# nlesc-smcm/hymls

Measured on AMD Instinct MI355X. Metric: Preconditioner ApplyInverse DoF/s + achieved HBM GB/s, Stokes3D, higher is better.
Workload: dtype f64

## Files before the change

hymls_amd/csrc/device.hpp:

```cpp
#pragma once
#include <cstdio>
#include "common.hpp"
#include "symbolic.hpp"

namespace hymls {
namespace dev {

struct Context;
Context* create_context(int device);
void bind(Context* c);
Context* current();
void destroy_context(Context* c);
void* stream();
const double* zeros16();
void* alloc(size_t bytes);
void free(void* p);
void h2d(void* dst, const void* src, size_t bytes);
void d2h(void* dst, const void* src, size_t bytes);
void d2d(void* dst, const void* src, size_t bytes);
void zero(void* dst, size_t bytes);
void sync();
size_t mem_free();
void* shared_scratch(size_t bytes);
constexpr int NSIDE = 8;
inline int side_streams() {
  static const int n = std::getenv("HYMLS_MI_SIDE_STREAMS") ? std::max(1, std::min(NSIDE, std::atoi(std::getenv("HYMLS_MI_SIDE_STREAMS")))) : 4;
  return n;
}
void fork_streams();
void use_stream(int k);
void join_streams();
void range_push(const char* label);
void range_pop();
struct Range {
  Range(const char* cls, int level, const char* fn) {
    char buf[96];
    std::snprintf(buf, sizeof buf, "%s_L%d: %s", cls, level, fn);
    range_push(buf);
  }
  ~Range() { range_pop(); }
  Range(const Range&) = delete;
  Range& operator=(const Range&) = delete;
};
void timer_start(int id);
double timer_stop(int id);
void mark(int phase, bool begin);
void profile_collect(double* sum, int* cnt);

template <class T, class A>
T* upload(const std::vector<T, A>& v) {
  T* p = (T*)alloc(std::max<size_t>(v.size(), 1) * sizeof(T));
  if (!v.empty()) h2d(p, v.data(), v.size() * sizeof(T));
  return p;
}

struct FrontD {
  int32_t c0, w, ri, rs;
  int32_t parent, idx_off, rel_off, c_off, a_off, lf_off;
  int32_t ent_begin, ent_end, child_begin, child_end;
  int64_t f_off, lp_off, q_off;
  int32_t pair = 0;
};

struct alignas(16) FwRec { int32_t item; uint16_t n; uint16_t s[5]; };

struct PlanD {
  int32_t nI, nS, nfronts, nent;
  const FrontD* fronts;
  const int32_t* fidx;
  const int32_t* rel;
  const int32_t* children;
  const int32_t* ent_id;
  const int32_t* ent_pos;
  const double* ent_w;
  const int32_t* asm_ptr;
  const int32_t* asm_src;
  int32_t asm_rows;
  const int32_t* fw_ptr;
  const int32_t* fw_items;
  const struct FwRec* fw_rec;
  const int32_t* bw_ptr;
  const int32_t* bw_items;
  int32_t nlev, max_level_rows;
  int32_t s_ent_begin, s_ent_end;
  int64_t scratch_size, factor_size;
  int32_t contrib_size;
  int32_t max_solve_rows;
  int32_t packed;
};

struct BatchD {
  int32_t nb;
  const int32_t* src;
  const int32_t* xoff;
  double* factor;
  double* scratch;
  double* sblock;
  double* contrib;
  int32_t* flag;
  double* tmp;
  int64_t tmp_stride;
  double* swork;
  int64_t swork_stride;
};

void gather(int64_t n, const int32_t* idx, const double* src, double* dst);
void scatter(int64_t n, const int32_t* idx, const double* src, double* dst);
void scatter_add(int64_t n, const int32_t* idx, const double* src, double* dst);
void axpby(int64_t n, double a, const double* x, double b, double* y);
void scale_copy(int64_t n, double a, const double* x, double* y);
inline int spmv_lanes(int32_t nrows, int64_t nnz_hint) {
  const double avg = nnz_hint >= 0 ? (double)nnz_hint / nrows : 8.0;
  return avg < 2.5 ? 1 : (avg < 5.0 ? 2 : (avg < 20.0 ? 4 : 8));
}
void spmv(int32_t nrows, const int32_t* rowptr, const int32_t* col, const double* val,
          const double* x, double* y, double alpha, double beta, int64_t nnz_hint = -1);
void spmv_mv(int32_t nrows, const int32_t* rowptr, const int32_t* col, const double* val, const double* x, int64_t ldx,
             double* y, int64_t ldy, int nv, double alpha, double beta, int64_t nnz_hint = -1);
void pull_sum(int64_t n, const int64_t* ptr, const int64_t* idx, const double* in, double* out);
void offdiag_count(int64_t nrows, const int32_t* rows, const int32_t* krow, const int32_t* kcol, const int32_t* ta, const int32_t* tb,
                   const int32_t* excl, int32_t* count);
void offdiag_fill(int64_t nrows, const int32_t* rows, const int32_t* krow, const int32_t* kcol, const int32_t* ta, const int32_t* tb,
                  const int32_t* excl, const int32_t* rowptr, int32_t* col, int32_t* src);
void member_sources(int32_t nb, int32_t next, int32_t nent, const int32_t* ext, const int32_t* ent_row, const int32_t* ent_col,
                    const int32_t* krow, const int32_t* kcol, int32_t* src, int32_t* flag);
void build_pull_tables(int64_t nrows, const int64_t* rcount, const int32_t* rowptr, const uint64_t* keys, int64_t* ptr, int64_t* idx);
void pull_sum_blocks(int64_t blen, int32_t nblk, const int64_t* ptr, const int64_t* base,
                     const double* in, double* out);

void factor_level(const PlanD& P, const BatchD& B, const int32_t* list, int32_t count,
                  int32_t b0, int32_t nbc, const double* kval, int32_t max_w);
void sblock_init(const PlanD& P, const BatchD& B, int32_t b0, int32_t nbc, const double* kval);

constexpr int PIECE = 128;
void factor_big_front(const PlanD& P, const BatchD& B, const FrontD& F, const FrontD* kids, int32_t nkids,
                      int32_t b0, int32_t nbc, const double* kval);
void root_update(const PlanD& P, const BatchD& B, const FrontD& F, int32_t nbc);
inline int solve_kt() {
  static const int kt = (std::getenv("HYMLS_MI_SOLVE_KT") && std::atoi(std::getenv("HYMLS_MI_SOLVE_KT")) == 1024) ? 1024 : 256;
  return kt;
}
void solve_fwd_big(const PlanD& P, const BatchD& B, const int32_t* list, const FrontD* hfronts, const int64_t* poff,
                   int32_t count, double* x);
void solve_bwd_big(const PlanD& P, const BatchD& B, const int32_t* list, const FrontD* hfronts, const int64_t* poff,
                   int32_t count, double* x);

void solve_fwd_level(const PlanD& P, const BatchD& B, const int32_t* list, int32_t count, double* x);
void solve_bwd_level(const PlanD& P, const BatchD& B, const int32_t* list, int32_t count, double* x);

#if defined(__HIPCC__)
#define HYMLS_HD __host__ __device__
#else
#define HYMLS_HD
#endif
HYMLS_HD inline int64_t packed_lower(int64_t w, int64_t i, int64_t k) { return k * (2 * w - k - 1) / 2 + (i - k - 1); }
HYMLS_HD inline int64_t packed_l21(int64_t w, int64_t ri, int64_t i, int64_t k) { return w * (w - 1) / 2 + i + ri * k; }
HYMLS_HD inline int64_t packed_upper(int64_t w, int64_t ri, int64_t i, int64_t k) { return w * (w - 1) / 2 + ri * w + k * (k + 1) / 2 + i; }
constexpr int32_t PAIR_L = 1, PAIR_Q = 2;
HYMLS_HD inline int64_t paired_cols(int64_t ld, int64_t ncol, int64_t i, int64_t k) {
  return k < (ncol & ~(int64_t)1) ? 2 * (ld * (k >> 1) + i) + (k & 1) : ld * k + i;
}
HYMLS_HD inline int64_t paired_lower(int64_t w, int64_t i, int64_t k) {
  const int64_t j = k >> 1;
  return i >= 2 * j + 2 ? 2 * j * (w - 1 - j) + 2 * (i - 2 * j - 2) + (k & 1) : w * (w - 1) / 2 - w / 2 + j;
}
HYMLS_HD inline int64_t paired_l21(int64_t w, int64_t ri, int64_t i, int64_t k) { return w * (w - 1) / 2 + paired_cols(ri, w, i, k); }
HYMLS_HD inline int64_t paired_q(int64_t w, int64_t ri, int64_t i, int64_t k) { return paired_cols(w, ri, i, k); }
void repack_fronts(const PlanD& P, const BatchD& B, int32_t b0, int32_t nbc);

struct FusedSub {
  union {
    const double* fac;
    const float* fac32;
  };
  int32_t xoff;
  int32_t cls;
};
constexpr int FUSED_MAX_ITEMS = 2048;
struct FusedIO {
  int32_t in = 0, out = 0, a_lanes = 1;
  const double* b = nullptr; const int32_t* perm = nullptr;
  const int32_t* a_row = nullptr; const int32_t* a_col = nullptr; const double* a_val = nullptr; const double* x2 = nullptr;
  const double* z = nullptr; double* user = nullptr;
};
void interior_solve_fused(int32_t nsub, const FusedSub* subs, const PlanD* plans, int32_t lds_doubles, double* x,
                          const FusedIO* io = nullptr);

constexpr int32_t FLAG_F32_RANGE = 4;
void demote_panels(int64_t n, const double* src, float* dst, int32_t* flag);
void round_panels(int64_t n, double* slab, int32_t* flag);
void interior_solve_fused_f32(int32_t nsub, const FusedSub* subs, const PlanD* plans, int32_t lds_doubles, double* x,
                              const FusedIO* io = nullptr);

struct LvlSub {
  union {
    const double* fac;
    const float* fac32;
  };
  double* contrib; int32_t xoff, cls;
  int64_t cstride;
};
struct LvlTask { int32_t sub, front, r0, pad; };
constexpr int LVL_MAX_ROWS = 6144;
constexpr int LVL_SMALL_ROWS = 256;
void solve_fwd_tasks(const LvlTask* tasks, int32_t ntasks, const LvlSub* subs, const PlanD* plans, int32_t lds_doubles,
                     const double* x, double* y);
void solve_bwd_tasks(const LvlTask* tasks, int32_t ntasks, const LvlSub* subs, const PlanD* plans, int32_t lds_doubles,
                     const double* y, double* x);

constexpr int NV_MAX = 4;
void interior_solve_fused_mv(int32_t nsub, const FusedSub* subs, const PlanD* plans, int32_t lds_doubles, int32_t front_doubles,
                             double* x, int64_t ldx, int nv);
void interior_solve_fused_mv_f32(int32_t nsub, const FusedSub* subs, const PlanD* plans, int32_t lds_doubles, int32_t front_doubles,
                                 double* x, int64_t ldx, int nv);
void solve_fwd_tasks_mv(const LvlTask* tasks, int32_t ntasks, const LvlSub* subs, const PlanD* plans, int32_t lds_doubles,
                        const double* x, double* y, int64_t ld, int nv);
void solve_bwd_tasks_mv(const LvlTask* tasks, int32_t ntasks, const LvlSub* subs, const PlanD* plans, int32_t lds_doubles,
                        const double* y, double* x, int64_t ld, int nv);
void solve_fwd_tasks_mv_f32(const LvlTask* tasks, int32_t ntasks, const LvlSub* subs, const PlanD* plans, int32_t lds_doubles,
                            const double* x, double* y, int64_t ld, int nv);
void solve_bwd_tasks_mv_f32(const LvlTask* tasks, int32_t ntasks, const LvlSub* subs, const PlanD* plans, int32_t lds_doubles,
                            const double* y, double* x, int64_t ld, int nv);

void ot_apply(int32_t ng, const int32_t* gptr, const double* w, double* x);
void sblock_transform(int32_t nS, int32_t ng, const int32_t* gptr, const double* tv,
                      double* sblock, int32_t nbc);
void sblock_extract(int32_t nS, int64_t npick, const int32_t* pick, const double* sblock,
                    double* out, int64_t out_stride, int32_t nbc);
struct KeptD {
  int32_t nS, ngl;
  const int32_t* gptr; const int32_t* glink; const int32_t* goff; const int64_t* lboff; const int32_t* lblen;
};
void sblock_kept(const KeptD& K, const double* tv, const double* sblock, double* out, int64_t out_stride, int32_t nbc);
bool sblock_kept_fits(int32_t nS, int32_t ngl);
void dense_invert(int32_t nb, int32_t nblk, double* blocks, int32_t* flag);
bool dense_invert_blocked_order(int32_t nb);
void blocks_apply(int32_t nb, int32_t nblk, const double* binv, const int32_t* ids,
                  const double* x, double* y);

double dot(int64_t n, const double* x, const double* y);
void solve_transposed(const PlanD& P, const BatchD& B, const int32_t* order, int32_t nfronts, int32_t max_rows, double* x);
// ... 9 lines not shown
```

hymls_amd/csrc/device_hip.hip:

```cpp
#include <hip/hip_runtime.h>
#include <type_traits>
#include <dlfcn.h>
#include <chrono>
#include <cstring>
#include <cfloat>
#include <array>
#include <map>
#include <string>
#include <cstdio>
#include "device.hpp"

namespace hymls {
namespace dev {

#define HIP_CHECK(call)                                                                    \
  do {                                                                                     \
    hipError_t e_ = (call);                                                                \
    if (e_ != hipSuccess)                                                                  \
      throw ::hymls::Error(-3, std::string("HIP error: ") + hipGetErrorString(e_) + " at " + \
                                   __FILE__ + ":" + std::to_string(__LINE__));             \
  } while (0)

struct MarkRec { int phase; bool begin; hipEvent_t ev; };
struct Context {
// ... 2179 lines not shown
  const bool pl = (F.pair & PAIR_L) != 0, pq = (F.pair & PAIR_Q) != 0;
  double* Q = B.factor + (int64_t)b * P.factor_size + F.q_off;
  for (int64_t t = threadIdx.x; t < n; t += 256) tmp[t] = Lp[t];
  if (pq) for (int64_t t = threadIdx.x; t < w * ri; t += 256) tmp[n + t] = Q[t];
  __syncthreads();
  for (int64_t t = threadIdx.x; t < n; t += 256) {
    const int64_t i = t % ld, k = t / ld;
    const int64_t dst = i >= w ? (pl ? paired_l21(w, ri, i - w, k) : packed_l21(w, ri, i - w, k))
                               : (i > k ? (pl ? paired_lower(w, i, k) : packed_lower(w, i, k)) : packed_upper(w, ri, i, k));
    Lp[dst] = tmp[t];
  }
  if (pq) for (int64_t t = threadIdx.x; t < w * ri; t += 256) Q[paired_q(w, ri, t % w, t / w)] = tmp[n + t];
}
void repack_fronts(const PlanD& P, const BatchD& B, int32_t b0, int32_t nbc) {
  if (P.nfronts <= 0 || nbc <= 0) return;
  hipLaunchKernelGGL(k_repack, dim3(P.nfronts, nbc), dim3(256), 0, g_stream, P, B, b0);
  launch_check();
}

__global__ void __launch_bounds__(256) k_demote_panels(const double* __restrict__ src, float* __restrict__ dst, int64_t n, int64_t head,
                                                        int32_t* __restrict__ flag) {
  const int64_t tid = (int64_t)blockIdx.x * 256 + threadIdx.x, nthr = (int64_t)gridDim.x * 256;
  bool bad = false;
  auto cv = [&](double v) { bad |= !(fabs(v) <= (double)FLT_MAX); return (float)v; };
  const int64_t nq = (n - head) / 4;
  const double2* s2 = (const double2*)(src + head);
  float4* d4 = (float4*)(dst + head);
  for (int64_t q = tid; q < nq; q += nthr) {
    const double2 a = s2[2 * q], b = s2[2 * q + 1];
    d4[q] = make_float4(cv(a.x), cv(a.y), cv(b.x), cv(b.y));
  }
  for (int64_t t = tid; t < head; t += nthr) dst[t] = cv(src[t]);
  for (int64_t t = head + 4 * nq + tid; t < n; t += nthr) dst[t] = cv(src[t]);
  if (bad) atomicOr(flag, FLAG_F32_RANGE);
}
void demote_panels(int64_t n, const double* src, float* dst, int32_t* flag) {
  if (n <= 0) return;
  int64_t head = std::min<int64_t>(n, (int64_t)(((16 - (uintptr_t)dst % 16) % 16) / sizeof(float)));
  if ((uintptr_t)(src + head) % 16 != 0) head = n;
  hipLaunchKernelGGL(k_demote_panels, dim3(nblocks(std::max<int64_t>(n / 4, 1), 256, 8192)), dim3(256), 0, g_stream, src, dst, n, head, flag);
  launch_check();
}
__global__ void __launch_bounds__(256) k_round_panels(double* __restrict__ slab, int64_t n, int32_t* __restrict__ flag) {
  bool bad = false;
  for (int64_t t = (int64_t)blockIdx.x * 256 + threadIdx.x; t < n; t += (int64_t)gridDim.x * 256) {
    const double v = slab[t];
    bad |= !(fabs(v) <= (double)FLT_MAX);
    slab[t] = (double)(float)v;
  }
  if (bad) atomicOr(flag, FLAG_F32_RANGE);
}
void round_panels(int64_t n, double* slab, int32_t* flag) {
  if (n <= 0) return;
  hipLaunchKernelGGL(k_round_panels, dim3(nblocks(n, 256, 8192)), dim3(256), 0, g_stream, slab, n, flag);
  launch_check();
}

struct FusedFront { int32_t c0, w, ri, c_off, a_off, lf_off, idx_off, pad; int64_t lp_off, q_off; };
template <class PTR>
__device__ inline PTR lside_pair(PTR base, int r, int w, int ri, int& c1, int& tri, PTR& ps) {
  const int low = (w * (w - 1)) >> 1;
  if (r < w) { c1 = 2 * (w - 3); tri = 1; ps = base + (low - (w >> 1) + ((r - 1) >> 1)); return base + (2 * r - 4); }
  c1 = 2 * ri; tri = 0; ps = base + (low + ri * (w - 1) + (r - w));
  return base + (low + 2 * (r - w));
}
template <class PTR>
__device__ inline PTR lside(PTR base, int packed, int r, int w, int ri, int& c1, int& tri) {
  if (!packed) { c1 = w + ri; tri = 0; return base + r; }
  if (r < w) { c1 = w; tri = 1; return base + (r - 1); }
  c1 = ri; tri = 0;
  return base + ((w * (w - 1)) >> 1) + (r - w);
}
template <class PTR>
__device__ inline PTR uside(PTR base, int packed, int i, int w, int ri, int& c1, int& tri) {
  if (!packed) { c1 = w + ri; tri = 0; return base + i; }
  c1 = 0; tri = 1;
  return base + ((w * (w - 1)) >> 1) + ri * w + i;
}
template <int L>
__device__ __forceinline__ void fused_spmv_rows(int n, int tid, gptr<int32_t> rp, gptr<int32_t> col, gptr<double> val, gptr<double> x, double* y) {
  const int lane = tid % L, rpb = 256 / L;
  for (int base = 0; base < n; base += 4 * rpb) {
    int k[4], e[4], c[4];
    double a[4], xv[4];
#pragma unroll
    for (int j = 0; j < 4; j++) {
      const int row = base + j * rpb + tid / L;
      k[j] = 0; e[j] = 0;
      if (row < n) { k[j] = rp[row] + lane; e[j] = rp[row + 1]; }
    }
#pragma unroll
    for (int j = 0; j < 4; j++) { a[j] = 0.0; c[j] = 0; if (k[j] < e[j]) { a[j] = val[k[j]]; c[j] = col[k[j]]; } }
#pragma unroll
    for (int j = 0; j < 4; j++) { xv[j] = 0.0; if (k[j] < e[j]) xv[j] = x[c[j]]; }
#pragma unroll
    for (int j = 0; j < 4; j++) {
      if (base + j * rpb >= n) break;
      const int row = base + j * rpb + tid / L;
      double s = 0.0;
      if (k[j] < e[j]) {
        s += a[j] * xv[j];
        for (int kk = k[j] + L; kk < e[j]; kk += L) s += val[kk] * x[col[kk]];
      }
#pragma unroll
      for (int off = L / 2; off > 0; off >>= 1) s += __shfl_down(s, off, L);
      if (row < n && lane == 0) y[row] = s + 0.0;
    }
  }
}
template <bool PROF, class PT, int IN, int OUT>
__device__ __forceinline__ void interior_fused_body(const FusedSub* __restrict__ subs, const PlanD* __restrict__ plans,
                                                    double* __restrict__ x, long long* __restrict__ prof, const FusedIO io) {
  extern __shared__ double lds[];
  auto ldp = [](gptr<PT> q) { return (double)*q; };
  long long tp[6] = {0, 0, 0, 0, 0, 0}, t0 = 0, tstart = 0;
  auto tick = [&](int bucket) { if (PROF) { const long long t = wall_clock64(); tp[bucket] += t - t0; t0 = t; } };
  if (PROF) { t0 = wall_clock64(); tstart = t0; }
  const FusedSub S = subs[blockIdx.x];
  const PlanD P = plans[S.cls];
  double* X = lds;
  double* C = lds + P.nI;
  double* Fv = C + P.contrib_size;
  double* R = Fv + 128;
  FusedFront* LF = (FusedFront*)(Fv + (P.max_level_rows > 384 ? P.max_level_rows : 384));
  const int tid = threadIdx.x;
  for (int i = tid; i < P.nfronts; i += 256) {
    const FrontD G = P.fronts[i];
    FusedFront f;
    f.c0 = G.c0; f.w = G.w; f.ri = G.ri; f.c_off = G.c_off; f.a_off = G.a_off; f.lf_off = G.lf_off; f.idx_off = G.idx_off;
    f.pad = P.packed ? G.pair : 0;
    f.lp_off = G.lp_off; f.q_off = G.q_off;
    LF[i] = f;
  }
  double* xg = x + S.xoff;
  if (IN == 0) {
    for (int i = tid; i < P.nI; i += 256) X[i] = xg[i];
  } else if (IN == 1) {
    const gptr<int32_t> perm = as_global(io.perm) + S.xoff;
    const gptr<double> b = as_global(io.b);
    for (int i = tid; i < P.nI; i += 256) X[i] = b[perm[i]];
  } else {
    const gptr<int32_t> a_row = as_global(io.a_row) + S.xoff, a_col = as_global(io.a_col);
    const gptr<double> a_val = as_global(io.a_val), x2 = as_global(io.x2);
    switch (io.a_lanes) {
      case 1: fused_spmv_rows<1>(P.nI, tid, a_row, a_col, a_val, x2, X); break;
      case 2: fused_spmv_rows<2>(P.nI, tid, a_row, a_col, a_val, x2, X); break;
      case 4: fused_spmv_rows<4>(P.nI, tid, a_row, a_col, a_val, x2, X); break;
      default: fused_spmv_rows<8>(P.nI, tid, a_row, a_col, a_val, x2, X); break;
    }
  }
  __syncthreads();
  tick(0);
  const gptr<PT> fac = as_global((const PT*)(const void*)S.fac);
  const gptr<int32_t> fw_items = as_global(P.fw_items), bw_items = as_global(P.bw_items), fidx = as_global(P.fidx),
                      asm_ptr = as_global(P.asm_ptr), asm_src = as_global(P.asm_src), fw_ptr = as_global(P.fw_ptr), bw_ptr = as_global(P.bw_ptr);
  typedef int v4i __attribute__((ext_vector_type(4)));
  const gptr<v4i> fw_rec = (gptr<v4i>)P.fw_rec;
  for (int lev = 0; lev < P.nlev; lev++) {
    const int ib = fw_ptr[lev], ni = fw_ptr[lev + 1] - ib;
    for (int it = tid; it < ni; it += 256) {
      FwRec rc;
      { const v4i q = fw_rec[ib + it]; static_assert(sizeof(FwRec) == 16, "FwRec is one dwordx4"); __builtin_memcpy(&rc, &q, 16); }
      const int item = rc.item;
      const FusedFront& F = LF[item >> 16];
      const int r = item & 0xffff;
      double v = r < F.w ? X[F.c0 + r] : 0.0;
      if (rc.n != 0xffff) {
#pragma unroll
        for (int q = 0; q < 5; q++) if (q < rc.n) v += C[rc.s[q]];
      } else {
        for (int t = asm_ptr[F.a_off + r]; t < asm_ptr[F.a_off + r + 1]; t++) v += C[asm_src[t]];
      }
      if (r < F.w) Fv[F.lf_off + r] = v; else C[F.c_off + r - F.w] = v;
    }
    __syncthreads();
    tick(1);
    if (ni > 128) {
      for (int it = tid; it < ni; it += 256) {
        const int item = fw_items[ib + it];
        const FusedFront& F = LF[item >> 16];
        const int r = item & 0xffff, w = F.w;
        int c1, tri;
        const double* f = Fv + F.lf_off;
        const int kmax = r < w ? r : w;
        double a[4];
#pragma unroll
        for (int u = 0; u < 4; u++) a[u] = 0.0;
        int k = 0;
        if (F.pad & PAIR_L) {
          gptr<PT> ps;
          const gptr<PT> pp = lside_pair(fac + F.lp_off, r, w, F.ri, c1, tri, ps);
          auto pair_at = [&](int j) { return load_pair<PT>(pp + (c1 * j - tri * 2 * j * j)); };
          for (; k + 3 < kmax; k += 4) {
            const PanelPair<PT> l0 = pair_at(k >> 1), l1 = pair_at((k >> 1) + 1);
            a[0] += (double)l0.a * f[k]; a[1] += (double)l0.b * f[k + 1]; a[2] += (double)l1.a * f[k + 2]; a[3] += (double)l1.b * f[k + 3];
          }
          const bool hp = k + 1 < kmax, hs = (kmax & 1) != 0;
          PanelPair<PT> tl = {}; PT ts = 0;
          if (hp) tl = pair_at(k >> 1);
          if (hs) ts = *ps;
          if (hp) { a[0] += (double)tl.a * f[k]; a[0] += (double)tl.b * f[k + 1]; }
          if (hs) a[0] += (double)ts * f[kmax - 1];
        } else {
          const gptr<PT> p = lside(fac + F.lp_off, P.packed, r, w, F.ri, c1, tri);
          for (; k + 3 < kmax; k += 4) {
            double l[4];
#pragma unroll
            for (int u = 0; u < 4; u++) l[u] = ldp(p + (c1 * (k + u) - tri * (((k + u) * (k + u + 3)) >> 1)));
#pragma unroll
            for (int u = 0; u < 4; u++) a[u] += l[u] * f[k + u];
          }
          tail_batch<3>([&](int u) { return k + u < kmax; },
                        [&](int u) { return ldp(p + (c1 * (k + u) - tri * (((k + u) * (k + u + 3)) >> 1))); },
                        [&](int u, double l) { a[0] += l * f[k + u]; });
        }
        const double sum = (a[0] + a[1]) + (a[2] + a[3]);
        if (r < w) X[F.c0 + r] = f[r] + sum; else C[F.c_off + r - w] -= sum;
      }
    } else {
      const int RT = ni > 64 ? 128 : 64, KG = 256 / RT;
      const int it = tid % RT, kg = tid / RT;
      double a0 = 0.0, a1 = 0.0, a2 = 0.0, a3 = 0.0;
      if (it < ni) {
        const int item = fw_items[ib + it];
        const FusedFront& F = LF[item >> 16];
        const int r = item & 0xffff, w = F.w;
        int c1, tri;
        const gptr<PT> p = lside(fac + F.lp_off, P.packed, r, w, F.ri, c1, tri);
        const double* f = Fv + F.lf_off;
        const int kmax = r < w ? r : w;
        auto at = [&](int kk) { return ldp(p + (c1 * kk - tri * ((kk * (kk + 3)) >> 1))); };
        int k = kg;
        for (; k + 3 * KG < kmax; k += 4 * KG) {
          const double l0 = at(k), l1 = at(k + KG), l2 = at(k + 2 * KG), l3 = at(k + 3 * KG);
          a0 += l0 * f[k]; a1 += l1 * f[k + KG]; a2 += l2 * f[k + 2 * KG]; a3 += l3 * f[k + 3 * KG];
        }
        tail_batch<3>([&](int u) { return k + u * KG < kmax; }, [&](int u) { return at(k + u * KG); },
                      [&](int u, double l) { a0 += l * f[k + u * KG]; });
      }
      R[kg * RT + it] = (a0 + a1) + (a2 + a3);
      __syncthreads();
      if (tid < ni) {
        const int item = fw_items[ib + tid];
        const FusedFront& F = LF[item >> 16];
        const int r = item & 0xffff;
        double sum = 0.0;
        for (int g = 0; g < KG; g++) sum += R[g * RT + tid];
        if (r < F.w) X[F.c0 + r] = Fv[F.lf_off + r] + sum; else C[F.c_off + r - F.w] -= sum;
      }
    }
    __syncthreads();
    tick(2);
  }
  for (int lev = P.nlev - 1; lev >= 0; lev--) {
    const int ib = bw_ptr[lev], ni = bw_ptr[lev + 1] - ib;
    if (ni > 128) {
      for (int it = tid; it < ni; it += 256) {
        const int item = bw_items[ib + it];
        const FusedFront& F = LF[item >> 16];
        const int i = item & 0xffff, w = F.w, ri = F.ri;
        int c1, tri;
        const gptr<PT> p = uside(fac + F.lp_off, P.packed, i, w, ri, c1, tri);
        const double* Xs = X + F.c0;
        double a[4];
#pragma unroll
        for (int u = 0; u < 4; u++) a[u] = 0.0;
        int k = i;
        for (; k + 3 < w; k += 4) {
          double l[4];
#pragma unroll
          for (int u = 0; u < 4; u++) l[u] = ldp(p + (c1 * (k + u) + tri * (((k + u) * (k + u + 1)) >> 1)));
#pragma unroll
          for (int u = 0; u < 4; u++) a[u] += l[u] * Xs[k + u];
        }
        tail_batch<3>([&](int u) { return k + u < w; },
                      [&](int u) { return ldp(p + (c1 * (k + u) + tri * (((k + u) * (k + u + 1)) >> 1))); },
                      [&](int u, double l) { a[0] += l * Xs[k + u]; });
        const gptr<int32_t> idx = fidx + F.idx_off + w;
        k = 0;
        if (F.pad & PAIR_Q) {
          const gptr<PT> qp = fac + F.q_off + 2 * i;
          for (; k + 3 < ri; k += 4) {
            const PanelPair<PT> l0 = load_pair<PT>(qp + w * k), l1 = load_pair<PT>(qp + w * (k + 2));
            int id[4];
#pragma unroll
            for (int u = 0; u < 4; u++) id[u] = idx[k + u];
            a[0] -= (double)l0.a * X[id[0]]; a[1] -= (double)l0.b * X[id[1]]; a[2] -= (double)l1.a * X[id[2]]; a[3] -= (double)l1.b * X[id[3]];
          }
          const bool hp = k + 1 < ri, hs = (ri & 1) != 0;
          PanelPair<PT> tl = {}; PT ts = 0; int i0 = 0, i1 = 0, i2 = 0;
          if (hp) { tl = load_pair<PT>(qp + w * k); i0 = idx[k]; i1 = idx[k + 1]; }
          if (hs) { ts = fac[F.q_off + w * (ri - 1) + i]; i2 = idx[ri - 1]; }
          if (hp) { a[0] -= (double)tl.a * X[i0]; a[0] -= (double)tl.b * X[i1]; }
          if (hs) a[0] -= (double)ts * X[i2];
        } else {
          const gptr<PT> qv = fac + F.q_off + i;
          for (; k + 3 < ri; k += 4) {
            double l[4]; int id[4];
#pragma unroll
            for (int u = 0; u < 4; u++) { l[u] = ldp(qv + (int64_t)w * (k + u)); id[u] = idx[k + u]; }
#pragma unroll
            for (int u = 0; u < 4; u++) a[u] -= l[u] * X[id[u]];
          }
          tail_batch<3>([&](int u) { return k + u < ri; },
                        [&](int u) { return QEntry{ldp(qv + (int64_t)w * (k + u)), idx[k + u]}; },
                        [&](int u, QEntry e) { a[0] -= e.q * X[e.id]; });
        }
        Fv[it] = (a[0] + a[1]) + (a[2] + a[3]);
      }
      __syncthreads();
      for (int it = tid; it < ni; it += 256) {
        const int item = bw_items[ib + it];
        X[LF[item >> 16].c0 + (item & 0xffff)] = Fv[it];
      }
    } else {
      const int RT = ni > 64 ? 128 : 64, KG = 256 / RT;
      const int it = tid % RT, kg = tid / RT;
      double a0 = 0.0, a1 = 0.0, a2 = 0.0, a3 = 0.0;
      if (it < ni) {
        const int item = bw_items[ib + it];
        const FusedFront& F = LF[item >> 16];
        const int i = item & 0xffff, w = F.w, ri = F.ri;
        int c1, tri;
        const gptr<PT> p = uside(fac + F.lp_off, P.packed, i, w, ri, c1, tri);
        const double* Xs = X + F.c0;
        auto at = [&](int kk) { return ldp(p + (c1 * kk + tri * ((kk * (kk + 1)) >> 1))); };
        int k = i + kg;
        for (; k + 3 * KG < w; k += 4 * KG) {
          const double l0 = at(k), l1 = at(k + KG), l2 = at(k + 2 * KG), l3 = at(k + 3 * KG);
          a0 += l0 * Xs[k]; a1 += l1 * Xs[k + KG]; a2 += l2 * Xs[k + 2 * KG]; a3 += l3 * Xs[k + 3 * KG];
        }
        tail_batch<3>([&](int u) { return k + u * KG < w; }, [&](int u) { return at(k + u * KG); },
                      [&](int u, double l) { a0 += l * Xs[k + u * KG]; });
        const gptr<PT> qv = fac + F.q_off + i;
        const gptr<int32_t> idx = fidx + F.idx_off + w;
        k = kg;
        for (; k + 3 * KG < ri; k += 4 * KG) {
          const double q0 = ldp(qv + (int64_t)w * k), q1 = ldp(qv + (int64_t)w * (k + KG)), q2 = ldp(qv + (int64_t)w * (k + 2 * KG)), q3 = ldp(qv + (int64_t)w * (k + 3 * KG));
          const int i0 = idx[k], i1 = idx[k + KG], i2 = idx[k + 2 * KG], i3 = idx[k + 3 * KG];
          a0 -= q0 * X[i0]; a1 -= q1 * X[i1]; a2 -= q2 * X[i2]; a3 -= q3 * X[i3];
        }
        tail_batch<3>([&](int u) { return k + u * KG < ri; },
                      [&](int u) { return QEntry{ldp(qv + (int64_t)w * (k + u * KG)), idx[k + u * KG]}; },
                      [&](int u, QEntry e) { a0 -= e.q * X[e.id]; });
      }
      R[kg * RT + it] = (a0 + a1) + (a2 + a3);
      __syncthreads();
      if (tid < ni) {
        const int item = bw_items[ib + tid];
        double sum = 0.0;
        for (int g = 0; g < KG; g++) sum += R[g * RT + tid];
        X[LF[item >> 16].c0 + (item & 0xffff)] = sum;
      }
    }
    __syncthreads();
    tick(ni > 128 ? 3 : 4);
  }
  if (OUT == 0) {
    for (int i = tid; i < P.nI; i += 256) xg[i] = X[i];
  } else {
    const gptr<int32_t> perm = as_global(io.perm) + S.xoff;
    const gptr<double> z = as_global(io.z) + S.xoff;
    const gmptr<double> user = as_global_rw(io.user);
    for (int i = tid; i < P.nI; i += 256) user[perm[i]] = z[i] - X[i];
  }
  if (PROF && tid == 0) {
    tp[5] = wall_clock64() - tstart;
    for (int q = 0; q < 6; q++) prof[(int64_t)blockIdx.x * 8 + q] = tp[q];
    prof[(int64_t)blockIdx.x * 8 + 6] = tstart;
    prof[(int64_t)blockIdx.x * 8 + 7] = P.nI;
  }
}
template <bool PROF, class PT>
__global__ void __launch_bounds__(256) __attribute__((amdgpu_waves_per_eu(8, 8))) k_interior_fused(const FusedSub* __restrict__ subs, const PlanD* __restrict__ plans,
                                                         double* __restrict__ x, long long* __restrict__ prof) {
  interior_fused_body<PROF, PT, 0, 0>(subs, plans, x, prof, FusedIO());
}
template <bool PROF, class PT, int IN, int OUT>
__global__ void __launch_bounds__(256) __attribute__((amdgpu_waves_per_eu(8, 8))) k_interior_fused_io(const FusedSub* __restrict__ subs, const PlanD* __restrict__ plans,
                                                            double* __restrict__ x, long long* __restrict__ prof, FusedIO io) {
  interior_fused_body<PROF, PT, IN, OUT>(subs, plans, x, prof, io);
}

template <bool PROF, class PT>
static void launch_fused_kernel(int32_t nsub, const FusedSub* subs, const PlanD* plans, size_t shm, double* x, long long* prof, const FusedIO& io) {
  auto go = [&](auto kernel, auto... tail) {
    if (shm > 64 * 1024) HIP_CHECK(hipFuncSetAttribute((const void*)kernel, hipFuncAttributeMaxDynamicSharedMemorySize, (int)shm));
    hipLaunchKernelGGL(kernel, dim3(nsub), dim3(256), shm, g_stream, subs, plans, x, prof, tail...);
  };
  if (io.in == 0 && io.out == 0) go(k_interior_fused<PROF, PT>);
  else if (io.in == 1 && io.out == 0) go(k_interior_fused_io<PROF, PT, 1, 0>, io);
  else if (io.in == 2 && io.out == 1) go(k_interior_fused_io<PROF, PT, 2, 1>, io);
  else HYMLS_CHECK(false, -3, "fused interior solve: no kernel for this combination of FusedIO::in and FusedIO::out");
  launch_check();
}
template <class PT>
static void launch_fused(int32_t nsub, const FusedSub* subs, const PlanD* plans, int32_t lds_doubles, double* x, const FusedIO* iop) {
  const FusedIO io = iop ? *iop : FusedIO();
  if (nsub <= 0) return;
  const size_t shm = (size_t)lds_doubles * sizeof(double);
  static const bool phase_prof = std::getenv("HYMLS_MI_FUSED_PROF") != nullptr;
  if (phase_prof) {
    long long* dprof = (long long*)alloc((size_t)nsub * 8 * sizeof(long long));
    launch_fused_kernel<true, PT>(nsub, subs, plans, shm, x, dprof, io);
    std::vector<long long> h((size_t)nsub * 8);
    d2h(h.data(), dprof, h.size() * sizeof(long long));
    free(dprof);
    double sum[6] = {0, 0, 0, 0, 0, 0};
    long long tmin = h[6], tmax = 0;
    for (int b = 0; b < nsub; b++) { for (int q = 0; q < 6; q++) sum[q] += (double)h[(size_t)b * 8 + q]; tmin = std::min(tmin, h[(size_t)b * 8 + 6]); tmax = std::max(tmax, h[(size_t)b * 8 + 6] + h[(size_t)b * 8 + 5]); }
    std::fprintf(stderr, "[hymls_mi] fused solve: %d workgroups, kernel span %.1f us; mean per workgroup (us): setup %.1f | fwd assembly %.1f | fwd panels %.1f | bwd panels (wide levels) %.1f | bwd panels (k-split levels) %.1f | total %.1f\n",
                 nsub, (tmax - tmin) / 100.0, sum[0] / nsub / 100, sum[1] / nsub / 100, sum[2] / nsub / 100, sum[3] / nsub / 100, sum[4] / nsub / 100, sum[5] / nsub / 100);
    return;
  }
  launch_fused_kernel<false, PT>(nsub, subs, plans, shm, x, nullptr, io);
}
void interior_solve_fused(int32_t nsub, const FusedSub* subs, const PlanD* plans, int32_t lds_doubles, double* x, const FusedIO* iop) {
  launch_fused<double>(nsub, subs, plans, lds_doubles, x, iop);
}
void interior_solve_fused_f32(int32_t nsub, const FusedSub* subs, const PlanD* plans, int32_t lds_doubles, double* x, const FusedIO* iop) {
  launch_fused<float>(nsub, subs, plans, lds_doubles, x, iop);
}

template <int NV, class PT>
__global__ void __launch_bounds__(256) k_interior_fused_mv(const FusedSub* __restrict__ subs, const PlanD* __restrict__ plans,
                                                            double* __restrict__ x, int64_t ldx) {
  extern __shared__ double lds[];
  const FusedSub S = subs[blockIdx.x];
  const PlanD P = plans[S.cls];
  const int nI = P.nI, CS = P.contrib_size, FS = P.max_level_rows > 384 ? P.max_level_rows : 384;
  double* X = lds;
  double* C = X + NV * nI;
  double* Fv = C + NV * CS;
  FusedFront* LF = (FusedFront*)(Fv + NV * FS);
  const int tid = threadIdx.x;
  for (int i = tid; i < P.nfronts; i += 256) {
    const FrontD G = P.fronts[i];
    FusedFront f;
    f.c0 = G.c0; f.w = G.w; f.ri = G.ri; f.c_off = G.c_off; f.a_off = G.a_off; f.lf_off = G.lf_off; f.idx_off = G.idx_off;
    f.pad = P.packed ? G.pair : 0;
    f.lp_off = G.lp_off; f.q_off = G.q_off;
    LF[i] = f;
  }
  double* xg = x + S.xoff;
#pragma unroll
  for (int v = 0; v < NV; v++)
    for (int i = tid; i < nI; i += 256) X[v * nI + i] = xg[v * ldx + i];
  __syncthreads();
  const gptr<PT> fac = as_global((const PT*)(const void*)S.fac);
  const gptr<int32_t> fw_items = as_global(P.fw_items), bw_items = as_global(P.bw_items), fidx = as_global(P.fidx),
                      asm_ptr = as_global(P.asm_ptr), asm_src = as_global(P.asm_src), fw_ptr = as_global(P.fw_ptr), bw_ptr = as_global(P.bw_ptr);
  typedef int v4i __attribute__((ext_vector_type(4)));
  const gptr<v4i> fw_rec = (gptr<v4i>)P.fw_rec;
  for (int lev = 0; lev < P.nlev; lev++) {
    const int ib = fw_ptr[lev], ni = fw_ptr[lev + 1] - ib;
    for (int it = tid; it < ni; it += 256) {
      FwRec rc;
      { const v4i q = fw_rec[ib + it]; __builtin_memcpy(&rc, &q, 16); }
      const int item = rc.item;
      const FusedFront& F = LF[item >> 16];
      const int r = item & 0xffff;
#pragma unroll
      for (int v = 0; v < NV; v++) {
        const double* Cv = C + v * CS;
        double val = r < F.w ? X[v * nI + F.c0 + r] : 0.0;
        if (rc.n != 0xffff) {
#pragma unroll
          for (int q = 0; q < 5; q++) if (q < rc.n) val += Cv[rc.s[q]];
        } else {
          for (int t = asm_ptr[F.a_off + r]; t < asm_ptr[F.a_off + r + 1]; t++) val += Cv[asm_src[t]];
        }
        if (r < F.w) Fv[v * FS + F.lf_off + r] = val; else C[v * CS + F.c_off + r - F.w] = val;
      }
    }
    __syncthreads();
    if (ni > 128) {
      for (int it = tid; it < ni; it += 256) {
        const int item = fw_items[ib + it];
        const FusedFront& F = LF[item >> 16];
        const int r = item & 0xffff, w = F.w;
        int c1, tri;
        const bool pl = (F.pad & PAIR_L) != 0;
        gptr<PT> ps = fac + F.lp_off;
        const gptr<PT> p = pl ? lside_pair(fac + F.lp_off, r, w, F.ri, c1, tri, ps) : lside(fac + F.lp_off, P.packed, r, w, F.ri, c1, tri);
        const double* f = Fv + F.lf_off;
        const int kmax = r < w ? r : w;
        auto at = [&](int kk) -> PT {
          if (!pl) return p[c1 * kk - tri * ((kk * (kk + 3)) >> 1)];
          const int j = kk >> 1;
          return kk < (kmax & ~1) ? p[c1 * j - tri * 2 * j * j + (kk & 1)] : *ps;
        };
        double a[4][NV];
#pragma unroll
        for (int u = 0; u < 4; u++)
#pragma unroll
          for (int v = 0; v < NV; v++) a[u][v] = 0.0;
        int k = 0;
// ... 869 lines not shown
```

hymls_amd/csrc/precond.cpp:

```cpp
#include "precond.hpp"
#include <cstring>
#include <chrono>
#include <thread>
#include <mutex>
#include <atomic>
#include <map>
#include <unordered_map>

namespace hymls {

namespace {

struct Hasher {
  uint64_t h = 1469598103934665603ULL;
  void add(const void* p, size_t n) {
    const unsigned char* c = (const unsigned char*)p;
    size_t i = 0;
    for (; i + 8 <= n; i += 8) {
      uint64_t w;
      std::memcpy(&w, c + i, 8);
      h = (h ^ w) * 0x9E3779B97F4A7C15ULL;
      h ^= h >> 29;
    }
    for (; i < n; i++) { h ^= c[i]; h *= 1099511628211ULL; }
  }
  template <class T> void addv(const std::vector<T>& v) { size_t n = v.size(); add(&n, sizeof n); if (n) add(v.data(), n * sizeof(T)); }
};

inline void gid_coord(const Params& p, int32_t gid, int32_t* c) {
  const int var = gid % p.dof, cell = gid / p.dof;
  const int i = cell % p.nx, j = (cell / p.nx) % p.ny, k = cell / (p.nx * p.ny);
  const int32_t vt = p.vtype[var];
  c[0] = 2 * i + (vt == VT_U); c[1] = 2 * j + (vt == VT_V); c[2] = 2 * k + (vt == VT_W);
}

constexpr int LEAF_SIZE = 24;
constexpr int LEAF_SIZE_UPPER = 64;
constexpr int MAX_WIDTH = 256;
constexpr int MAX_WIDTH_COARSE = 256;
constexpr int LEAF_SIZE_COARSE = 512;
static const int64_t SCRATCH_BUDGET = [] {
  const char* e = std::getenv("HYMLS_MI_SCRATCH_GIB");
  const double gib = e ? std::max(0.25, std::atof(e)) : 8.0;
  return (int64_t)(gib * (double)(1LL << 27));
}();

}

Csr drop_by_value(const Csr& A, double tol, int kind) {
  Csr R;
  drop_by_value(A, tol, kind, R);
  return R;
}

void drop_by_value(const Csr& A, double tol, int kind, Csr& R) {
  const bool zero_diag = kind == 1, full_diag = kind == 2;
  R.n = A.n;
  R.rowptr.resize(A.n + 1);
  R.rowptr[0] = 0;
  dvec diag(A.n, 0.0);
  parallel_for(A.n, [&](int64_t i) {
    double d = 0.0, rmax = 0.0;
    for (int e = A.rowptr[i]; e < A.rowptr[i + 1]; e++) {
      rmax = std::max(rmax, std::abs(A.val[e]));
      if (A.col[e] == i) d = A.val[e];
    }
    diag[i] = std::abs(d) <= tol * rmax ? 0.0 : d;
  });
  auto row = [&](int64_t i, int32_t* col, double* val) {
    int32_t n = 0;
    auto put = [&](int32_t j, double v) { if (col) { col[n] = j; val[n] = v; } n++; };
    if (full_diag) put((int32_t)i, std::abs(diag[i]) > tol ? diag[i] : 0.0);
    for (int e = A.rowptr[i]; e < A.rowptr[i + 1]; e++) {
      const int j = A.col[e];
      const bool isd = j == i;
      if (isd && full_diag) continue;
      const double scal = isd ? 1.0 : std::max(std::abs(diag[i]), std::abs(diag[j]));
      const double v = isd ? diag[i] : A.val[e];
      if (std::abs(v) > scal * tol && std::abs(v) > tol) put(j, v);
      else if (isd && zero_diag) put(j, 0.0);
    }
    return n;
  };
  parallel_for(A.n, [&](int64_t i) { R.rowptr[i + 1] = row(i, nullptr, nullptr); });
  for (int i = 0; i < A.n; i++) R.rowptr[i + 1] += R.rowptr[i];
  if (R.col.size() != (size_t)R.rowptr[A.n]) { cvec().swap(R.col); R.col.resize((size_t)R.rowptr[A.n]); }
  if (R.val.size() != (size_t)R.rowptr[A.n]) { vvec().swap(R.val); R.val.resize((size_t)R.rowptr[A.n]); }
  parallel_for(A.n, [&](int64_t i) { row(i, R.col.data() + R.rowptr[i], R.val.data() + R.rowptr[i]); });
}

BatchedLU::~BatchedLU() {
  for (void* p : owned) dev::free(p);
  dev::free(factor32);
}

void BatchedLU::release_factor() {
  if (!batch.factor) return;
  owned.erase(std::remove(owned.begin(), owned.end(), (void*)batch.factor), owned.end());
  dev::free(batch.factor);
  batch.factor = nullptr;
}
void BatchedLU::hold_factor() {
  if (batch.factor) return;
  batch.factor = (double*)dev::alloc(factor_bytes((int64_t)members.size(), plan.factor_size));
  owned.push_back(batch.factor);
}
void BatchedLU::hold_factor32() {
  if (!factor32) factor32 = (float*)dev::alloc(factor_bytes((int64_t)members.size(), plan.factor_size) / 2);
}
void BatchedLU::release_factor32() { dev::free(factor32); factor32 = nullptr; }
double BatchedLU::resident_bytes() const {
  const double fb = (double)factor_bytes((int64_t)members.size(), plan.factor_size);
  return (batch.factor ? fb : 0.0) + (factor32 ? fb / 2 : 0.0);
}

void BatchedLU::plan_scratch(int64_t budget, bool with_sblock) {
  const int nb = (int)members.size();
  const int64_t per = plan.scratch_size + (with_sblock ? (int64_t)plan.nS * plan.nS : 0);
  chunk = (int32_t)std::max<int64_t>(1, std::min<int64_t>(nb, budget / std::max<int64_t>(per, 1)));
  scratch_need_ = std::max<int64_t>(1, (int64_t)chunk * plan.scratch_size);
  sblock_need_ = with_sblock ? std::max<int64_t>(1, (int64_t)chunk * plan.nS * plan.nS) : 0;
  bool any_wide = false;
  for (auto& L : plan.fwide_levels) any_wide |= !L.empty();
  batch.tmp_stride = 0; tmp_need_ = 0;
  if (any_wide) {
    const int64_t np = (plan.max_w + dev::PIECE - 1) / dev::PIECE;
    batch.tmp_stride = np * 2 * dev::PIECE * dev::PIECE + 2LL * plan.max_w * dev::PIECE;
    tmp_need_ = (int64_t)chunk * batch.tmp_stride;
  }
}

void BatchedLU::upload(int64_t budget, bool with_sblock) {
  const int nb = (int)members.size();
  nent = (int32_t)plan.ent_id.size();
  std::vector<dev::FrontD> fd(plan.fronts.size());
  for (size_t s = 0; s < fd.size(); s++) {
    const Front& F = plan.fronts[s];
    fd[s] = dev::FrontD{F.c0, F.w, F.ri, F.rs, F.parent, F.idx_off, F.rel_off, F.c_off, F.a_off, F.lf_off,
                        F.ent_begin, F.ent_end, F.child_begin, F.child_end, F.f_off, F.lp_off, F.q_off};
  }
#ifdef HYMLS_MI_PAIRED_PANELS
  if (packed && (paired || std::getenv("HYMLS_MI_FORCE_PAIRED_PANELS"))) {
    for (size_t s = 0; s < fd.size(); s++) {
      const int32_t lev = plan.fronts[s].level;
      if (lev < 0 || lev + 1 >= (int32_t)plan.fw_ptr.size() || lev + 1 >= (int32_t)plan.bw_ptr.size()) continue;
      if (plan.fw_ptr[lev + 1] - plan.fw_ptr[lev] > 128) fd[s].pair |= dev::PAIR_L;
      if (plan.bw_ptr[lev + 1] - plan.bw_ptr[lev] > 128) fd[s].pair |= dev::PAIR_Q;
    }
  }
#endif
  auto keep = [&](auto* p) { owned.push_back((void*)p); return p; };
  dplan.nI = plan.nI; dplan.nS = plan.nS; dplan.nfronts = (int32_t)fd.size(); dplan.nent = nent;
  dplan.fronts = keep(dev::upload(fd));
  dplan.fidx = keep(dev::upload(plan.fidx));
  dplan.rel = keep(dev::upload(plan.rel));
  dplan.children = keep(dev::upload(plan.children));
  dplan.ent_id = keep(dev::upload(plan.ent_id));
  dplan.ent_pos = keep(dev::upload(plan.ent_pos));
  dplan.ent_w = keep(dev::upload(plan.ent_w));
  dplan.asm_ptr = keep(dev::upload(plan.asm_ptr));
  dplan.asm_src = keep(dev::upload(plan.asm_src));
  dplan.asm_rows = plan.asm_rows;
  dplan.fw_ptr = keep(dev::upload(plan.fw_ptr)); dplan.fw_items = keep(dev::upload(plan.fw_items));
  dplan.bw_ptr = keep(dev::upload(plan.bw_ptr)); dplan.bw_items = keep(dev::upload(plan.bw_items));
  {
    std::vector<dev::FwRec> rec(plan.fw_items.size());
    for (size_t t = 0; t < rec.size(); t++) {
      const int32_t item = plan.fw_items[t];
      const Front& F = plan.fronts[item >> 16];
      const int32_t a = F.a_off + (item & 0xffff);
      const int32_t nb = plan.asm_ptr[a], ne = plan.asm_ptr[a + 1];
      dev::FwRec r{item, (uint16_t)(ne - nb), {0, 0, 0, 0, 0}};
      if (ne - nb > 5 || plan.contrib_size > 65535) r.n = 0xffff;
      else for (int32_t q = nb; q < ne; q++) r.s[q - nb] = (uint16_t)plan.asm_src[q];
      rec[t] = r;
    }
    dplan.fw_rec = keep(dev::upload(rec));
  }
  dplan.nlev = (int32_t)plan.levels.size(); dplan.max_level_rows = plan.max_level_rows;
  dplan.s_ent_begin = plan.s_ent_begin; dplan.s_ent_end = nent;
  dplan.scratch_size = plan.scratch_size; dplan.factor_size = plan.factor_size;
  dplan.contrib_size = plan.contrib_size;
  dplan.packed = packed ? 1 : 0;
  {
    int32_t msr = 1;
    for (auto& F : plan.fronts) if (!F.big) msr = std::max(msr, F.w + F.ri);
    dplan.max_solve_rows = msr;
  }
  for (auto& L : plan.levels) d_lists.push_back(keep(dev::upload(L)));
  for (auto& L : plan.flevels) d_flists.push_back(keep(dev::upload(L)));
  plan_scratch(budget, with_sblock);
  batch.nb = nb;
  if (!h_ext.empty()) {
    HYMLS_CHECK(d_krow && d_kcol && (int64_t)h_ent_row.size() == nent && (int64_t)h_ext.size() == (int64_t)nb * n_ext, -3,
                "entry source lists: inconsistent tables");
    int32_t* src = (int32_t*)keep(dev::alloc(std::max<int64_t>(1, (int64_t)nb * nent) * sizeof(int32_t)));
    int32_t* d_ext = dev::upload(h_ext);
    int32_t* d_er = dev::upload(h_ent_row);
    int32_t* d_ec = dev::upload(h_ent_col);
    int32_t* d_fl = (int32_t*)dev::alloc(sizeof(int32_t));
    dev::zero(d_fl, sizeof(int32_t));
    dev::member_sources(nb, n_ext, nent, d_ext, d_er, d_ec, d_krow, d_kcol, src, d_fl);
    int32_t fl = 0;
    dev::d2h(&fl, d_fl, sizeof fl);
    dev::free(d_ext); dev::free(d_er); dev::free(d_ec); dev::free(d_fl);
    HYMLS_CHECK(fl == 0, -3, "entry of a subdomain pattern not found in the level matrix");
    batch.src = src;
    { rawvec<int32_t>().swap(h_ext); }
  } else {
    batch.src = keep(dev::upload(h_src));
  }
  batch.xoff = keep(dev::upload(h_xoff));
  const size_t fbytes = factor_bytes(nb, plan.factor_size);
  batch.factor = (double*)keep(pre_factor && pre_factor->bytes == fbytes ? pre_factor->take() : dev::alloc(fbytes));
  pre_factor.reset();
  batch.scratch = nullptr; batch.sblock = nullptr;
  batch.contrib = (double*)keep(dev::alloc(std::max<int64_t>(1, (int64_t)contrib_nv * nb * plan.contrib_size) * sizeof(double)));
  batch.flag = (int32_t*)keep(dev::alloc(4 * sizeof(int32_t)));
  dev::zero(batch.flag, 4 * sizeof(int32_t));
  h_fronts = fd;
  bool any_big = false, any_wide = false;
  for (auto& L : plan.big_levels) any_big |= !L.empty();
  for (auto& L : plan.fwide_levels) any_wide |= !L.empty();
  batch.tmp = nullptr; batch.swork = nullptr; batch.swork_stride = 0;
  (void)any_wide;
  if (any_big) {
    int64_t part_max = 0;
    for (auto& L : plan.big_levels) {
      d_big_lists.push_back(keep(dev::upload(L)));
      h_big_fronts.emplace_back();
      std::vector<int64_t> poff;
      int64_t off = 0;
      for (int s : L) {
        h_big_fronts.back().push_back(fd[s]);
        const int64_t w = fd[s].w, ri = fd[s].ri, kt = dev::solve_kt();
        const int64_t ctw = (w + kt - 1) / kt, ctr = (ri + kt - 1) / kt;
        poff.push_back(off);
        off += std::max(ctw * (w + ri), (ctw + ctr) * w);
      }
      part_max = std::max(part_max, off);
      d_big_poff.push_back(keep(dev::upload(poff)));
    }
    batch.swork_stride = (int64_t)plan.asm_rows + part_max;
    batch.swork = (double*)keep(dev::alloc((size_t)nb * batch.swork_stride * sizeof(double)));
  }
}

std::vector<dev::FrontD> BatchedLU::kids_of(int s) const {
  std::vector<dev::FrontD> k;
  for (int e = plan.fronts[s].child_begin; e < plan.fronts[s].child_end; e++) k.push_back(h_fronts[plan.children[e]]);
  return k;
}

void BatchedLU::bind_scratch() {
  double* a = (double*)dev::shared_scratch((size_t)(scratch_need_ + sblock_need_ + tmp_need_) * sizeof(double));
  batch.scratch = a;
  batch.sblock = sblock_need_ ? a + scratch_need_ : nullptr;
  batch.tmp = tmp_need_ ? a + scratch_need_ + sblock_need_ : nullptr;
}

void BatchedLU::factor_chunk(const double* kval, int32_t b0, int32_t nbc, bool spread_wide) {
  bind_scratch();
  if (batch.sblock) dev::sblock_init(dplan, batch, b0, nbc, kval);
  const bool spread = spread_wide && dev::side_streams() > 1 && !std::getenv("HYMLS_MI_NO_SIDE_STREAMS");
  struct MainStreamGuard { bool on; ~MainStreamGuard() { if (on) { try { dev::use_stream(0); } catch (...) {} } } } back_to_main{spread};
  for (size_t l = 0; l < plan.flevels.size(); l++) {
    int32_t mw = 1;
    for (int s : plan.flevels[l]) mw = std::max(mw, plan.fronts[s].w);
    dev::factor_level(dplan, batch, d_flists[l], (int32_t)plan.flevels[l].size(), b0, nbc, kval, mw);
    const auto& wide = plan.fwide_levels[l];
    if (spread && wide.size() > 1) {
      dev::fork_streams();
      for (size_t q = 0; q < wide.size(); q++) {
        dev::use_stream(1 + (int)(q % dev::side_streams()));
        dev::BatchD bq = batch;
        bq.tmp = tmp_need_ ? (double*)dev::shared_scratch((size_t)tmp_need_ * sizeof(double)) : nullptr;
        auto k = kids_of(wide[q]);
        dev::factor_big_front(dplan, bq, h_fronts[wide[q]], k.data(), (int32_t)k.size(), b0, nbc, kval);
      }
      dev::join_streams();
      continue;
    }
    for (int s : wide) {
      auto k = kids_of(s);
      dev::factor_big_front(dplan, batch, h_fronts[s], k.data(), (int32_t)k.size(), b0, nbc, kval);
    }
  }
  if (batch.sblock)
    for (size_t s = 0; s < plan.fronts.size(); s++)
      if (!plan.fronts[s].wide && plan.fronts[s].parent < 0 && plan.fronts[s].rs > 0) dev::root_update(dplan, batch, h_fronts[s], nbc);
}

void BatchedLU::repack_chunk(int32_t b0, int32_t nbc) {
  if (packed) dev::repack_fronts(dplan, batch, b0, nbc);
}

void BatchedLU::solve(double* x) const {
  const int nl = (int)plan.levels.size();
  for (int l = 0; l < nl; l++) {
    dev::solve_fwd_level(dplan, batch, d_lists[l], (int32_t)plan.levels[l].size(), x);
    if (!plan.big_levels[l].empty())
      dev::solve_fwd_big(dplan, batch, d_big_lists[l], h_big_fronts[l].data(), d_big_poff[l], (int32_t)plan.big_levels[l].size(), x);
  }
  for (int l = nl - 1; l >= 0; l--) {
    if (!plan.big_levels[l].empty())
      dev::solve_bwd_big(dplan, batch, d_big_lists[l], h_big_fronts[l].data(), d_big_poff[l], (int32_t)plan.big_levels[l].size(), x);
    dev::solve_bwd_level(dplan, batch, d_lists[l], (int32_t)plan.levels[l].size(), x);
  }
}

int32_t BatchedLU::check_flag(double* growth) const {
  int32_t f[4] = {0, 0, 0, 0};
  dev::d2h(f, batch.flag, sizeof f);
  if (growth) std::memcpy(growth, f + 2, sizeof(double));
  return f[0];
}

bool merged_solve_fits(const ClassPlan& plan) {
  for (auto& F : plan.fronts) if (F.w + F.ri > dev::LVL_MAX_ROWS) return false;
  return true;
}

FusedNeed fused_solve_need(const ClassPlan& plan) {
  const int32_t fronts = (int32_t)(plan.fronts.size() * 6 + 1);
  return FusedNeed{plan.nI + plan.contrib_size + std::max(plan.max_level_rows, 384) + fronts, fronts};
}

bool fused_solve_fits(const ClassPlan& plan) {
  constexpr int32_t LDS_CAP = 12288;
  bool any_big = false;
// ... 2296 lines not shown
```

Baseline: 2.639 billion.

## Pre-gather backward-solve update values into contiguous contribution buffer per level

In the fused backward triangular solve, each level now starts with a gather pass that copies the needed solution entries from X into the per-front contribution area C, using packed (dst<<16|src) records precomputed on the host. The inner update loops then read C contiguously instead of loading an index from global memory and doing an indirect LDS read per entry. This drops the global index traffic and the dependent indirection from the hot loop. In exchange it adds a gather pass and an extra barrier per level, and it is limited to 16-bit offsets, which are checked on the host.

```diff
diff --git a/hymls_amd/csrc/device.hpp b/hymls_amd/csrc/device.hpp
--- a/hymls_amd/csrc/device.hpp
+++ b/hymls_amd/csrc/device.hpp
@@ -87,6 +87,8 @@
   int32_t contrib_size;
   int32_t max_solve_rows;
   int32_t packed;
+  const int32_t* bg_ptr = nullptr;
+  const int32_t* bg_rec = nullptr;
 };
 
 struct BatchD {
diff --git a/hymls_amd/csrc/device_hip.hip b/hymls_amd/csrc/device_hip.hip
--- a/hymls_amd/csrc/device_hip.hip
+++ b/hymls_amd/csrc/device_hip.hip
@@ -2355,7 +2355,7 @@
   __syncthreads();
   tick(0);
   const gptr<PT> fac = as_global((const PT*)(const void*)S.fac);
-  const gptr<int32_t> fw_items = as_global(P.fw_items), bw_items = as_global(P.bw_items), fidx = as_global(P.fidx),
+  const gptr<int32_t> fw_items = as_global(P.fw_items), bw_items = as_global(P.bw_items), bg_ptr = as_global(P.bg_ptr), bg_rec = as_global(P.bg_rec),
                       asm_ptr = as_global(P.asm_ptr), asm_src = as_global(P.asm_src), fw_ptr = as_global(P.fw_ptr), bw_ptr = as_global(P.bw_ptr);
   typedef int v4i __attribute__((ext_vector_type(4)));
   const gptr<v4i> fw_rec = (gptr<v4i>)P.fw_rec;
@@ -2457,6 +2457,14 @@
   }
   for (int lev = P.nlev - 1; lev >= 0; lev--) {
     const int ib = bw_ptr[lev], ni = bw_ptr[lev + 1] - ib;
+    const int gb = bg_ptr[lev], gn = bg_ptr[lev + 1] - gb;
+    if (gn > 0) {
+      for (int t = tid; t < gn; t += 256) {
+        const uint32_t rec = (uint32_t)bg_rec[gb + t];
+        C[rec >> 16] = X[rec & 0xffff];
+      }
+      __syncthreads();
+    }
     if (ni > 128) {
       for (int it = tid; it < ni; it += 256) {
         const int item = bw_items[ib + it];
@@ -2479,35 +2487,32 @@
         tail_batch<3>([&](int u) { return k + u < w; },
                       [&](int u) { return ldp(p + (c1 * (k + u) + tri * (((k + u) * (k + u + 1)) >> 1))); },
                       [&](int u, double l) { a[0] += l * Xs[k + u]; });
-        const gptr<int32_t> idx = fidx + F.idx_off + w;
+        const double* Ca = C + F.c_off;
         k = 0;
         if (F.pad & PAIR_Q) {
           const gptr<PT> qp = fac + F.q_off + 2 * i;
           for (; k + 3 < ri; k += 4) {
             const PanelPair<PT> l0 = load_pair<PT>(qp + w * k), l1 = load_pair<PT>(qp + w * (k + 2));
-            int id[4];
-#pragma unroll
-            for (int u = 0; u < 4; u++) id[u] = idx[k + u];
-            a[0] -= (double)l0.a * X[id[0]]; a[1] -= (double)l0.b * X[id[1]]; a[2] -= (double)l1.a * X[id[2]]; a[3] -= (double)l1.b * X[id[3]];
+            a[0] -= (double)l0.a * Ca[k]; a[1] -= (double)l0.b * Ca[k + 1]; a[2] -= (double)l1.a * Ca[k + 2]; a[3] -= (double)l1.b * Ca[k + 3];
           }
           const bool hp = k + 1 < ri, hs = (ri & 1) != 0;
-          PanelPair<PT> tl = {}; PT ts = 0; int i0 = 0, i1 = 0, i2 = 0;
-          if (hp) { tl = load_pair<PT>(qp + w * k); i0 = idx[k]; i1 = idx[k + 1]; }
-          if (hs) { ts = fac[F.q_off + w * (ri - 1) + i]; i2 = idx[ri - 1]; }
-          if (hp) { a[0] -= (double)tl.a * X[i0]; a[0] -= (double)tl.b * X[i1]; }
-          if (hs) a[0] -= (double)ts * X[i2];
+          PanelPair<PT> tl = {}; PT ts = 0;
+          if (hp) tl = load_pair<PT>(qp + w * k);
+          if (hs) ts = fac[F.q_off + w * (ri - 1) + i];
+          if (hp) { a[0] -= (double)tl.a * Ca[k]; a[0] -= (double)tl.b * Ca[k + 1]; }
+          if (hs) a[0] -= (double)ts * Ca[ri - 1];
         } else {
           const gptr<PT> qv = fac + F.q_off + i;
           for (; k + 3 < ri; k += 4) {
-            double l[4]; int id[4];
-#pragma unroll
-            for (int u = 0; u < 4; u++) { l[u] = ldp(qv + (int64_t)w * (k + u)); id[u] = idx[k + u]; }
-#pragma unroll
-            for (int u = 0; u < 4; u++) a[u] -= l[u] * X[id[u]];
+            double l[4];
+#pragma unroll
+            for (int u = 0; u < 4; u++) l[u] = ldp(qv + (int64_t)w * (k + u));
+#pragma unroll
+            for (int u = 0; u < 4; u++) a[u] -= l[u] * Ca[k + u];
           }
           tail_batch<3>([&](int u) { return k + u < ri; },
-                        [&](int u) { return QEntry{ldp(qv + (int64_t)w * (k + u)), idx[k + u]}; },
-                        [&](int u, QEntry e) { a[0] -= e.q * X[e.id]; });
+                        [&](int u) { return ldp(qv + (int64_t)w * (k + u)); },
+                        [&](int u, double q) { a[0] -= q * Ca[k + u]; });
         }
         Fv[it] = (a[0] + a[1]) + (a[2] + a[3]);
       }
@@ -2536,16 +2541,15 @@
         tail_batch<3>([&](int u) { return k + u * KG < w; }, [&](int u) { return at(k + u * KG); },
                       [&](int u, double l) { a0 += l * Xs[k + u * KG]; });
         const gptr<PT> qv = fac + F.q_off + i;
-        const gptr<int32_t> idx = fidx + F.idx_off + w;
+        const double* Ca = C + F.c_off;
         k = kg;
         for (; k + 3 * KG < ri; k += 4 * KG) {
           const double q0 = ldp(qv + (int64_t)w * k), q1 = ldp(qv + (int64_t)w * (k + KG)), q2 = ldp(qv + (int64_t)w * (k + 2 * KG)), q3 = ldp(qv + (int64_t)w * (k + 3 * KG));
-          const int i0 = idx[k], i1 = idx[k + KG], i2 = idx[k + 2 * KG], i3 = idx[k + 3 * KG];
-          a0 -= q0 * X[i0]; a1 -= q1 * X[i1]; a2 -= q2 * X[i2]; a3 -= q3 * X[i3];
+          a0 -= q0 * Ca[k]; a1 -= q1 * Ca[k + KG]; a2 -= q2 * Ca[k + 2 * KG]; a3 -= q3 * Ca[k + 3 * KG];
         }
         tail_batch<3>([&](int u) { return k + u * KG < ri; },
-                      [&](int u) { return QEntry{ldp(qv + (int64_t)w * (k + u * KG)), idx[k + u * KG]}; },
-                      [&](int u, QEntry e) { a0 -= e.q * X[e.id]; });
+                      [&](int u) { return ldp(qv + (int64_t)w * (k + u * KG)); },
+                      [&](int u, double q) { a0 -= q * Ca[k + u * KG]; });
       }
       R[kg * RT + it] = (a0 + a1) + (a2 + a3);
       __syncthreads();
diff --git a/hymls_amd/csrc/precond.cpp b/hymls_amd/csrc/precond.cpp
--- a/hymls_amd/csrc/precond.cpp
+++ b/hymls_amd/csrc/precond.cpp
@@ -176,6 +176,35 @@
       rec[t] = r;
     }
     dplan.fw_rec = keep(dev::upload(rec));
+  }
+  dplan.bg_ptr = dplan.bg_rec = nullptr;
+  if (fused_solve_fits(plan)) {
+    const int32_t nl = (int32_t)plan.levels.size();
+    std::vector<int32_t> owner((size_t)plan.nI, -1);
+    for (size_t s = 0; s < plan.fronts.size(); s++)
+      for (int32_t t = 0; t < plan.fronts[s].w; t++) owner[plan.fronts[s].c0 + t] = (int32_t)s;
+    std::vector<int32_t> ptr(1, 0), rec;
+    for (int32_t l = 0; l < nl; l++) {
+      std::vector<std::pair<int32_t, int32_t>> ranges;
+      for (int s : plan.levels[l]) {
+        const Front& F = plan.fronts[s];
+        if (F.ri == 0) continue;
+        ranges.emplace_back(F.c_off, F.ri);
+        for (int32_t k = 0; k < F.ri; k++) {
+          const int32_t dst = F.c_off + k, src = plan.fidx[F.idx_off + F.w + k];
+          HYMLS_CHECK(dst >= 0 && dst < plan.contrib_size && dst < 65536, -3, "fused solve gather: contribution entry out of range");
+          HYMLS_CHECK(src >= 0 && src < plan.nI && src < 65536, -3, "fused solve gather: update row outside the interior");
+          HYMLS_CHECK(owner[src] >= 0 && plan.fronts[owner[src]].level > l, -3, "fused solve gather: update row not owned by a higher level");
+          rec.push_back((int32_t)(((uint32_t)dst << 16) | (uint32_t)src));
+        }
+      }
+      std::sort(ranges.begin(), ranges.end());
+      for (size_t q = 1; q < ranges.size(); q++)
+        HYMLS_CHECK(ranges[q - 1].first + ranges[q - 1].second <= ranges[q].first, -3, "fused solve gather: contribution vectors of one level overlap");
+      ptr.push_back((int32_t)rec.size());
+    }
+    dplan.bg_ptr = keep(dev::upload(ptr));
+    dplan.bg_rec = keep(dev::upload(rec));
   }
   dplan.nlev = (int32_t)plan.levels.size(); dplan.max_level_rows = plan.max_level_rows;
   dplan.s_ent_begin = plan.s_ent_begin; dplan.s_ent_end = nent;
```

Result: faster. 2.681 billion, median of 6 (+1.6%).
